# SJTU-ViSYS/Ground-Fusion

Measured on AMD Instinct MI355X. Metric: sliding-window solves/sec + tracked-features/sec, 640x480x10-frame window, higher is better.
Workload: dtype front end u8/s16 fixed point + f32; back end f64

## Files before the change

ground-fusion_amd/csrc/gf_ba.hip:

```cpp
#pragma clang fp contract(fast)
#include <hip/hip_runtime.h>
#include <algorithm>
#include <cmath>
#include <cstdio>
#include <cstdlib>
#include <cstring>
#include <atomic>
#include <memory>
#include <mutex>
#include <string>
#include <thread>
#include <vector>

#include "../../include/groundfusion_hip.h"
#include "gf_comm.hpp"
#include "gf_ba_kernels.hpp"
#include "gf_copy_list.hpp"
#include "gf_ba_marg.hpp"
#include "gf_ba_gnss.hpp"
#include "gf_hip_own.hpp"

using namespace gfb;

__global__ void ba_fill_plausible(void* p, size_t i0, size_t i1, int is_double, unsigned seed) {
// ... 658 lines not shown
}

int run_solve(gf_ba* h, int max_iters) {
    const Dims& d = h->d;
    const auto t_begin = std::chrono::steady_clock::now();
    if (int rc = launch_linearize(h, 0, 0, 0, false)) return rc;
    Win w = h->win();
    StepBufs sb = h->sbufs();
    const bool fuse_misc = h->fuse_misc && h->can_fuse_misc && d.GO == 0 && h->n_chain == 0;
    for (int it = 0; it <= max_iters; it++) {
        if (h->max_solver_time > 0.0 && it > 0 && it < max_iters) {
            HIPCHK(hipStreamSynchronize(h->stream));
            if (std::chrono::duration<double>(std::chrono::steady_clock::now() - t_begin).count() >= h->max_solver_time) it = max_iters;
        }
        poison_lds(h);
        const bool time_step = it == 1 && max_iters >= 1;
        if (time_step) HIPCHK(hipEventRecord(h->ev[6], h->stream));
        const int first = it == 0 ? 1 : 0, last = it == max_iters ? 1 : 0;
        const LaunchForm& ch = h->step_chain; const LaunchForm& de = h->step_dense;
        if (h->n_chain > 0) ch.fn<<<dim3(d.B), ch.threads, ch_lds_doubles(h->chain_nd) * sizeof(double), h->stream>>>(w, sb, first, max_iters, last);
        if (h->n_chain > 0 && h->n_dense == 0) { }
        else if (fuse_misc && it > 0 && h->step_waves != 4) ba_misc_step<<<dim3(d.B), 512, std::max(h->step_lds, h->mwin_lds), h->stream>>>(w, sb, max_iters, last);
        else de.fn<<<dim3(d.B), de.threads, de.lds, h->stream>>>(w, sb, first, max_iters, last);
        HIPCHK(hipGetLastError());
        if (time_step) { HIPCHK(hipEventRecord(h->ev[7], h->stream)); h->stats.step_launches++; h->stats.step_flops += h->step_flops; }
        if (it < max_iters) {
            const bool cost_only = h->cost_only && it == max_iters - 1 && it > 0 && d.GO == 0 && !h->split_jtj && !fuse_misc && !(h->max_solver_time > 0.0);
            if (int rc = launch_linearize(h, -1, -1, cost_only ? 3 : 1, it == 0, fuse_misc)) return rc;
            if (it == 0) { h->stats.jtj_launches++; h->stats.jtj_flops += h->mfma_per_lin * 2048; h->stats.jtj_alg_flops += h->jtj_alg_flops; }
        }
    }
    h->stats.solves += h->count;
    return GF_OK;
}

int run_marginalize(gf_ba* h, int mode) {
    const Dims& d = h->d;
    Win w = h->win();
    poison_lds(h);
    Win wm = w;
    wm.colf = h->mcolf[mode].d; wm.cole = h->mcole[mode].d; wm.order = h->morder[mode].d; wm.norder = h->mnorder[mode].d;
    if (mode == 0) { if (int rc = launch_visual(h, wm, true, -1, -2, 2)) return rc; }
    ba_linearize_misc_win<<<dim3(d.B), 64 * kMW, h->mwin_lds, h->stream>>>(wm, -1, -2, 2, mode == 0 ? 1 : 2);
    if (mode == 0 && d.GO) ba_linearize_gnss<<<dim3(d.B), 256, 0, h->stream>>>(wm, -1, -2, 2, 1);
    MargOut mo{h->outJ.d, h->outr.d};
    const double piv_eps = h->piv_eps;
    const int ls_rhs = h->ls_rhs;
    poison_lds(h);
    if (h->big_marg) ba_marg_finish<true><<<dim3(d.B), 512, 0, h->stream>>>(wm, h->sbufs(), reinterpret_cast<const MargInfo*>(h->minfo[mode].d), mo, mode == 0 ? 1 : 0, piv_eps, ls_rhs, 0);
    else ba_marg_finish<false><<<dim3(d.B), 512, h->marg_lds, h->stream>>>(wm, h->sbufs(), reinterpret_cast<const MargInfo*>(h->minfo[mode].d), mo, mode == 0 ? 1 : 0, piv_eps, ls_rhs, (int)(h->marg_lds / sizeof(double)));
    HIPCHK(hipGetLastError());
    return GF_OK;
}

}

extern "C" {

int gf_pose_subset_mask(int extrinsic_type) {
    switch (extrinsic_type) {
        case 0: return 0x00;
        case 2: return 0x07;
        case 3: return 0x04;
        case 4: return 0x3c;
        default: return 0x38;
    }
}

int gf_ba_create(const gf_ba_cfg* cfg, gf_ba** out) {
    if (!cfg || !out) return gf::set_err(GF_ERR_INVALID, "null argument");
    *out = nullptr;
    if (cfg->window_size < 2 || cfg->window_size > 30 || cfg->max_features < 1 || cfg->max_visual < 1 || cfg->batch < 1) return gf::set_err(GF_ERR_INVALID, "bad gf_ba_cfg");
    if (int rc = gf::require_device()) return rc;
    std::unique_ptr<gf_ba> h(new gf_ba());
    h->cfg = *cfg;
    Dims& d = h->d;
    d.B = cfg->batch; d.W = cfg->window_size; d.NP = d.W + 1; d.F = cfg->max_features; d.NV = cfg->max_visual;
    d.NVP = ((d.NV + d.NP * d.NP / 2 + 63) / 64) * 64;
    const bool gnss = cfg->max_gnss > 0;
    d.NG = gnss ? ((cfg->max_gnss + 63) & ~63) : 0; d.NGRP = gnss ? 4 * d.NP : 0;
    const int Rmax = 15 * d.NP + 17 + (gnss ? 5 * d.NP + 3 : 0);
    d.RP = (Rmax + 1 + 15) & ~15;  d.GO = gnss ? ((16 * d.NP + 20 + d.F + 3) & ~3) : 0; d.XS = gnss ? ((d.GO + 5 * d.NP + 4 + 3) & ~3) : ((16 * d.NP + 20 + d.F + 3) & ~3); d.NFB = 2 * d.NP + 7 + (gnss ? 5 * d.NP + 2 : 0); d.FP = (d.F + 3) & ~3; d.NPRI = d.RP; d.ECW = (6 * d.NP + 8 + 15) & ~15; d.NC = 6 * d.NP + 8; d.NVC = (d.NC * (d.NC + 1) / 2 + 3) & ~3;
    h->step_lds = (size_t)(Rmax + 1) * (Rmax + 2) / 2 * sizeof(double);
    h->big_step = h->step_lds + 27 * 1024 > 160 * 1024 || getenv("GF_BA_FORCE_GLOBAL") != nullptr;
    if (Rmax + 1 > 512) return gf::set_err(GF_ERR_INVALID, "window_size %d: reduced system (%d) exceeds 511 columns", d.W, Rmax);
    if (d.NV > 65535) return gf::set_err(GF_ERR_INVALID, "max_visual %d exceeds 65535", d.NV);
    if (misc_win_lds_doubles(d.W) * sizeof(double) > 160 * 1024)  return gf::set_err(GF_ERR_INVALID, "window_size %d: the IMU / wheel block rows exceed LDS (window_size <= 20 in this build)", d.W);
#define TRACED(x) do { g_alloc_what = #x; if (int rc_ = (x)) return rc_; } while (0)
    {
        int least = 0, greatest = 0;
        HIPCHK(hipDeviceGetStreamPriorityRange(&least, &greatest));
        const char* e = getenv("GF_BA_STREAM_PRIORITY");
        const int prio = (e && !strcmp(e, "default")) ? least + (greatest - least) / 2 : greatest;
        HIPCHK(hipStreamCreateWithPriority(&h->stream.s, hipStreamNonBlocking, prio));
    }
    for (auto& e : h->ev) HIPCHK(hipEventCreate(&e.e));
    HIPCHK(hipEventCreateWithFlags(&h->ev_gather.e, hipEventDisableTiming));
    HIPCHK(hipEventCreateWithFlags(&h->ev_gather_done.e, hipEventDisableTiming));
    const size_t B = d.B, VS = d.RP + d.FP;
    TRACED(h->xs0.alloc(B * d.XS, true)); TRACED(h->xs.alloc(2 * B * d.XS, true));
    TRACED(h->colf.alloc(B * d.NFB, true)); TRACED(h->cole.alloc(B * d.F, true)); TRACED(h->nvis.alloc(B, true)); TRACED(h->nimu.alloc(B, true)); TRACED(h->nwh.alloc(B, true)); TRACED(h->nfeat.alloc(B, true));
    TRACED(h->vis_idx.alloc(B * d.NV, true)); TRACED(h->vis_data.alloc(B * d.NV * 5, true)); TRACED(h->feat_obs.alloc(B * d.F * 6, true));
    TRACED(h->order.alloc(B * d.NVP, true)); TRACED(h->norder.alloc(B, true)); TRACED(h->feat_ptr.alloc(B * (d.F + 1), true)); TRACED(h->vis_pos.alloc(B * d.NV, true));
    TRACED(h->imu_i.alloc(B * d.W, true)); TRACED(h->imu_data.alloc(B * d.W * IMU_STRIDE2, true)); TRACED(h->wh_i.alloc(B * d.W, true)); TRACED(h->wh_data.alloc(B * d.W * WH_STRIDE, true));
    TRACED(h->pri_n.alloc(B, true)); TRACED(h->pri_nb.alloc(B, true)); TRACED(h->pri_bid.alloc(B * 64, true)); TRACED(h->pri_J.alloc(B * d.NPRI * d.NPRI, true));
    TRACED(h->pri_r.alloc(B * d.NPRI, true)); TRACED(h->pri_x0.alloc(B * d.NPRI * 2, true));
    HIPCHK(h->st.dev.alloc(B)); HIPCHK(h->st.pin.alloc(B)); h->st.view();
    HIPCHK(h->st0.dev.alloc(B)); HIPCHK(h->st0.pin.alloc(B)); h->st0.view();
    h->upload_kernel = !(getenv("GF_BA_UPLOAD") && !strcmp(getenv("GF_BA_UPLOAD"), "copies"));
    TRACED(h->imu_sqrt.alloc(B * d.W * 225, false)); TRACED(h->wh_sqrt.alloc(B * d.W * 36, false)); TRACED(h->pri_A.alloc(B * d.NPRI * d.NPRI, false)); TRACED(h->pri_b.alloc(B * d.NPRI, false));
    TRACED(h->pri_c.alloc(B, false)); TRACED(h->H.alloc(2 * B * d.RP * d.RP, true)); TRACED(h->g.alloc(2 * B * d.RP, true)); TRACED(h->Vc.alloc(2 * B * d.NVC, true)); TRACED(h->wpar.alloc(B * WPAR, true));
    TRACED(h->cost.alloc(6 * B, true)); TRACED(h->efac.alloc(B * d.NV * EF, false));
    HIPCHK(hipMemsetAsync(h->cost.d, 0, 6 * B * sizeof(double), h->stream));
    TRACED(h->scale.alloc(B * VS, false)); TRACED(h->diag.alloc(B * VS, false)); TRACED(h->grad.alloc(B * VS, false)); TRACED(h->gn.alloc(B * VS, false)); TRACED(h->step.alloc(B * VS, false));
    TRACED(h->u.alloc(B * VS, false)); TRACED(h->Et.alloc(2 * B * d.FP * d.ECW, true)); TRACED(h->Es.alloc(B * d.FP * d.ECW, false)); TRACED(h->ete.alloc(2 * B * d.FP, true)); TRACED(h->etb.alloc(2 * B * d.FP, true));
    TRACED(h->rhs.alloc(B * d.RP, false)); TRACED(h->yv.alloc(B * VS, false));
    if (gnss) { TRACED(h->ngnss.alloc(B, true)); TRACED(h->gn_idx.alloc(B * d.NG * 4, true)); TRACED(h->gn_data.alloc(B * d.NG * GN_STRIDE, true)); TRACED(h->gn_misc.alloc(B * (GN_MISC + d.NP), true)); TRACED(h->gn_gptr.alloc(B * (d.NGRP + 2), true)); TRACED(h->gn_gitem.alloc(B * d.NG, true)); TRACED(h->gn_rows.alloc(B * d.NG * GN_ROW, false)); }
    for (int m = 0; m < 2; m++) { TRACED(h->mcolf[m].alloc(B * d.NFB, true)); TRACED(h->mcole[m].alloc(B * d.F, true)); TRACED(h->morder[m].alloc(B * d.NVP, true)); TRACED(h->mnorder[m].alloc(B, true)); TRACED(h->minfo[m].alloc(B * 4, true)); }
    TRACED(h->minfo_stage.alloc(B * 4, true));
    TRACED(h->vpair.alloc(B * (size_t)(d.NP * (d.NP - 1) / 2) * VPG, false));
    TRACED(h->outJ.alloc(B * (size_t)d.NPRI * d.NPRI, true)); TRACED(h->outr.alloc(B * d.NPRI, true)); TRACED(h->stamps.alloc(128, true));
    const int nkeep = 6 * d.W + 9 + 17 + (gnss ? 9 : 0);
    h->big_marg = nkeep > 92 || getenv("GF_BA_FORCE_GLOBAL") != nullptr;
    h->meta.assign(d.B, gf_ba::SlotMeta{}); h->outJ_n.assign(d.B, 0); h->imu_dev.assign(d.B, 0); h->imu_rows.assign(d.B, 0);
    TRACED(h->imu_patch.alloc(B * d.W * IMU_STRIDE2, true)); TRACED(h->imu_pinfo.alloc(B * (d.W + 2), true));
    for (int mode = 0; mode < 2; mode++) h->keep_ids[mode].assign(d.B, {});
    h->marg_ncap = h->big_marg ? std::min(d.NPRI, nkeep + 16) : 92;
    h->marg_lds = h->big_marg ? 0 : (size_t)2 * h->marg_ncap * h->marg_ncap * sizeof(double);
    if (h->big_step) { h->sg_stride = (h->step_lds / sizeof(double) + 15) & ~(size_t)15; TRACED(h->Sg.alloc(B * h->sg_stride, false)); }
    if (h->big_marg) { h->mg_stride = (size_t)2 * h->marg_ncap * h->marg_ncap + 1024; TRACED(h->Mg.alloc(B * h->mg_stride, false)); }
    if (getenv("GF_BA_SPLIT_JTJ") && atoi(getenv("GF_BA_SPLIT_JTJ"))) if (int rc = gf_ba_set_split_jtj(h.get(), 1)) return rc;
    h->step_waves = (getenv("GF_BA_STEP_WAVES") && atoi(getenv("GF_BA_STEP_WAVES")) == 4) ? 4 : 8;
    h->chain_mode = getenv("GF_BA_CHAIN") && atoi(getenv("GF_BA_CHAIN")) != 0 && !h->big_step && !gnss;
    h->cost_only = !(getenv("GF_BA_COST_ONLY") && atoi(getenv("GF_BA_COST_ONLY")) == 0);
    h->piv_eps = getenv("GF_MARG_PIVOT_EPS") ? atof(getenv("GF_MARG_PIVOT_EPS")) : 3e-8;
    h->ls_rhs = getenv("GF_MARG_LS_RHS") ? atoi(getenv("GF_MARG_LS_RHS")) : 1;
    const int nd_max = Rmax - 9 * d.NP;
    if (h->chain_mode && ch_lds_doubles(nd_max) * sizeof(double) + 20 * 1024 > 160 * 1024) h->chain_mode = false;
    if (int rc = choose_launch_forms(h.get(), nd_max)) return rc;
    if (h->chain_mode) { h->yg_stride = ch_y_stride(nd_max); TRACED(h->Yg.alloc(B * d.NP * h->yg_stride, false)); }
    h->fuse_misc = getenv("GF_BA_FUSE_MISC") != nullptr;
    if (!h->vis_fixed.lds || !h->vis_free.lds) { h->vtile_stride = (vwin_slot_doubles(d.NP, true) + 3) & ~(size_t)3; TRACED(h->vtile.alloc(B * h->vtile_stride, false)); }
    h->mwin_lds = misc_win_lds_doubles(d.W) * sizeof(double);
    HIPCHK(hipFuncSetAttribute(reinterpret_cast<const void*>(ba_linearize_misc_win), hipFuncAttributeMaxDynamicSharedMemorySize, (int)h->mwin_lds));
    h->can_fuse_misc = !h->big_step && std::max(h->step_lds, h->mwin_lds) + 27 * 1024 <= 160 * 1024;
    if (h->can_fuse_misc) HIPCHK(hipFuncSetAttribute(reinterpret_cast<const void*>(ba_misc_step), hipFuncAttributeMaxDynamicSharedMemorySize, (int)std::max(h->step_lds, h->mwin_lds)));
    if (!h->big_marg) HIPCHK(hipFuncSetAttribute(reinterpret_cast<const void*>(ba_marg_finish<false>), hipFuncAttributeMaxDynamicSharedMemorySize, (int)h->marg_lds));
    HIPCHK(hipStreamSynchronize(h->stream));
#undef TRACED
    *out = h.release();
    return GF_OK;
}

int gf_ba_destroy(gf_ba* h) { delete h; return GF_OK; }

int gf_ba_upload(gf_ba* h, const gf_ba_window* windows, int count) {
    if (!h || !windows) return gf::set_err(GF_ERR_INVALID, "null argument");
    if (int rc = gf_ba_wait(h)) return rc;
    std::fill(h->outJ_n.begin(), h->outJ_n.end(), 0);
    if (int rc = pack_windows(h, windows, count)) return rc;
    h->resident.assign(count, nullptr);
    for (int b = 0; b < count; b++) h->resident[b] = windows + b;
    HIPCHK(hipEventRecord(h->ev[0], h->stream));
    if (int rc = upload(h)) return rc;
    HIPCHK(hipEventRecord(h->ev[1], h->stream));
    HIPCHK(hipStreamSynchronize(h->stream));
    float ms = 0; HIPCHK(hipEventElapsedTime(&ms, h->ev[0], h->ev[1])); h->stats.ms_upload += ms;
    return GF_OK;
}

int gf_ba_solve_resident_async(gf_ba* h, int max_iters, int marginalize_mode, int reset) {
    if (!h || h->count < 1) return gf::set_err(GF_ERR_INVALID, "no resident windows");
    if (h->pending) return gf::set_err(GF_ERR_INVALID, "a solve is already in flight: call gf_ba_wait first");
    if (max_iters < 0 || max_iters > 64) return gf::set_err(GF_ERR_INVALID, "max_iters out of range");
    if (marginalize_mode > 1) return gf::set_err(GF_ERR_INVALID, "marginalize_mode must be -1, 0 or 1");
    if (reset) { if (int rc = reset_state(h)) return rc; }
    HIPCHK(hipEventRecord(h->ev[0], h->stream));
    if (int rc = run_solve(h, max_iters)) return rc;
    HIPCHK(hipEventRecord(h->ev[1], h->stream));
    if (marginalize_mode >= 0) { if (int rc = run_marginalize(h, marginalize_mode)) return rc; h->last_marg_mode = marginalize_mode; }
    HIPCHK(hipEventRecord(h->ev[4], h->stream));
    h->pending = true; h->pending_iters = max_iters;
    return GF_OK;
}

int gf_ba_wait(gf_ba* h) {
    if (!h) return gf::set_err(GF_ERR_INVALID, "null handle");
    if (!h->pending) return GF_OK;
    HIPCHK(hipStreamSynchronize(h->stream));
    h->pending = false;
    float ms = 0;
    HIPCHK(hipEventElapsedTime(&ms, h->ev[0], h->ev[1])); h->stats.ms_solve += ms;
    HIPCHK(hipEventElapsedTime(&ms, h->ev[1], h->ev[4])); h->stats.ms_marginalize += ms;
    if (h->pending_iters > 0) { HIPCHK(hipEventElapsedTime(&ms, h->ev[2], h->ev[3])); h->stats.ms_jtj += ms; }
    if (h->pending_iters > 0 && h->split_timed) { HIPCHK(hipEventElapsedTime(&ms, h->ev_split[0], h->ev_split[1])); h->stats.ms_jtj_contract += ms; h->stats.jtj_contract_launches++; h->split_timed = false; }
    if (h->pending_iters > 0) { HIPCHK(hipEventElapsedTime(&ms, h->ev[6], h->ev[7])); h->stats.ms_step += ms; }
    return GF_OK;
}

int gf_ba_solve_resident(gf_ba* h, int max_iters, int marginalize_mode, int reset) {
    if (int rc = gf_ba_solve_resident_async(h, max_iters, marginalize_mode, reset)) return rc;
    return gf_ba_wait(h);
}


static int unpack_prior(gf_ba* h, int b, int mode, const double* x, gf_ba_prior& p) {
    const Dims& d = h->d;
    const int* inf = h->minfo[mode].h + (size_t)b * 4;
    p.valid = inf[3]; p.m = inf[0] + inf[1]; p.n = 0; p.nblocks = 0;
    if (!inf[3]) return GF_OK;
    const int n = inf[2];
    const std::vector<int>& keep = h->keep_ids[mode][b];
    if (n > p.cap_n || (int)keep.size() > p.cap_blocks) return gf::set_err(GF_ERR_CAPACITY, "prior capacity too small (n=%d, blocks=%zu)", n, keep.size());
    p.n = n; p.nblocks = (int)keep.size();
    if (p.J) memcpy(p.J, h->outJ.h + (size_t)b * d.NPRI * d.NPRI, (size_t)n * n * sizeof(double));
    memcpy(p.r, h->outr.h + (size_t)b * d.NPRI, (size_t)n * sizeof(double));
    int xo = 0;
    for (size_t q = 0; q < keep.size(); q++) {
        const int id = keep[q], kind = id / 4096, i = id % 4096;
        int nid = id;
        if (kind == GF_POSE || kind == GF_SPEEDBIAS || kind == GF_RCV_DDT) nid = mode == 0 ? kind * 4096 + i - 1 : (i == d.W ? kind * 4096 + d.W - 1 : id);
        else if (kind == GF_RCV_DT) nid = mode == 0 ? id - 4 : (i / 4 == d.W ? id - 4 : id);
        p.block_id[q] = nid;
        const int off = state_off_of(id, d);
        for (int k = 0; k < gsize_kind(kind); k++) p.x0[xo++] = x[off + k];
    }
    return GF_OK;
}
// ... 220 lines not shown
```

ground-fusion_amd/csrc/gf_ba_kernels.hpp:

```cpp
#pragma once
#include <type_traits>
#include <hip/hip_runtime.h>
#include <stdint.h>
#include "gf_dmath.hpp"

namespace gfb {
using namespace gfd;

typedef double d4 __attribute__((ext_vector_type(4)));

struct Dims {
    int B, W, NP, F, NV, NVP, RP, XS, NFB, FP, NPRI, ECW, GO, NG, NC, NVC, NGRP;
};
__host__ __device__ inline int off_pose(int i) { return 16 * i; }
__host__ __device__ inline int off_sb(int i) { return 16 * i + 7; }
__host__ __device__ inline int off_ex(int NP) { return 16 * NP; }
__host__ __device__ inline int off_exw(int NP) { return 16 * NP + 7; }
__host__ __device__ inline int off_ix(int NP) { return 16 * NP + 14; }
__host__ __device__ inline int off_td(int NP) { return 16 * NP + 17; }
__host__ __device__ inline int off_tdw(int NP) { return 16 * NP + 18; }
__host__ __device__ inline int off_feat(int NP) { return 16 * NP + 20; }
__host__ __device__ inline int fb_pose(int i) { return 2 * i; }
__host__ __device__ inline int fb_sb(int i) { return 2 * i + 1; }
__host__ __device__ inline int fb_ex(int NP) { return 2 * NP; }
// ... 1279 lines not shown
        a[J] = l;
        asm("" : "+v"(r));
        if (r == J) rd_own = rs;
        const double nlw = (r > J) ? -(l * rs) : 0.0;
        if (J > 0) Chol16W<J, 0>::fence(t);
        Chol16W<J, 0>::run(t, nlw);
        if (J < N - 1) {
            double nl = -l;
            dpp_fence(nl);
            Chol16A<J, J + 1, N>::run(a, nl, l);
        }
        Chol16Step<J + 1, N>::run(a, t, r, rd_own, good);
    }
};
template <int N> struct Chol16Step<N, N> { static __device__ __forceinline__ void run(double (&)[16], double (&)[4], int&, double&, bool&) {} };
template <class SPtr>
__device__ __forceinline__ bool wave_chol16_fused(SPtr S, int j0, int nb, double* s_inv, int lane) {
    int r = lane & 15;
    const int g = lane >> 4;
    double a[16], t[4];
    {
        const int base = pk(j0 + min(r, nb - 1), j0);
#pragma unroll
        for (int c = 0; c < 16; c++) a[c] = S[base + c];
        if (nb < 16) {
#pragma unroll
            for (int c = 0; c < 16; c++) a[c] = (r < nb && c < nb) ? a[c] : (r == c ? 1.0 : 0.0);
        }
    }
#pragma unroll
    for (int m = 0; m < 4; m++) t[m] = (4 * m + g == r) ? 1.0 : 0.0;
    double rd_own = 0.0;
    bool good = true;
    Chol16Step<0>::run(a, t, r, rd_own, good);
#pragma unroll
    for (int m = 0; m < 4; m++) {
        const int c = 4 * m + g;
        const double w = t[m] * rd_own;
        s_inv[r * 17 + c] = w;
        if (c <= r && r < nb) S[pk(j0 + r, j0 + c)] = w;
    }
    __builtin_amdgcn_fence(__ATOMIC_RELEASE, "wavefront"); __builtin_amdgcn_wave_barrier();
    return good;
}

__device__ __forceinline__ int ch_dm(int c, int NP) { return c < 15 * NP ? 6 * (c / 15) + (c % 15) : c - 9 * NP; }
__device__ __forceinline__ int ch_d2c(int dj, int NP) { return dj < 6 * NP ? 15 * (dj / 6) + dj % 6 : dj + 9 * NP; }
__device__ __forceinline__ bool ch_isv(int c, int NP) { return c < 15 * NP && (c % 15) >= 6; }
constexpr int kChPS = 13;
constexpr int kChYS = 9;
__host__ __device__ inline int ch_panel_rows(int ND) { return (ND + 1 + 15) & ~15; }
__host__ __device__ inline size_t ch_lds_doubles(int ND) { return (((size_t)(ND + 1) * (ND + 2) / 2 + 1) & ~(size_t)1) + 2 * (size_t)ch_panel_rows(ND) * kChPS + 3 * 272; }
__host__ __device__ inline size_t ch_y_stride(int ND) { return (size_t)ch_panel_rows(ND) * kChYS + 2 * 81; }
template <int NB, int LD>
__device__ __forceinline__ bool wave_chol_tile(const double* sA, double* s_inv, int lane) {
    int r = lane & 15;
    const int g = lane >> 4;
    double a[16], t[4];
    {
        const double* src = sA + min(r, NB - 1) * LD;
#pragma unroll
        for (int c = 0; c < 16; c++) a[c] = c < NB ? src[c] : 0.0;
#pragma unroll
        for (int c = 0; c < 16; c++) a[c] = (r < NB && c < NB) ? a[c] : (r == c ? 1.0 : 0.0);
    }
#pragma unroll
    for (int m = 0; m < 4; m++) t[m] = (4 * m + g == r) ? 1.0 : 0.0;
    double rd_own = 1.0;
    bool good = true;
    Chol16Step<0, NB>::run(a, t, r, rd_own, good);
#pragma unroll
    for (int m = 0; m < 4; m++) s_inv[r * 17 + 4 * m + g] = t[m] * rd_own;
    __builtin_amdgcn_fence(__ATOMIC_RELEASE, "wavefront"); __builtin_amdgcn_wave_barrier();
    return good;
}

template <bool GS, int NW = 8, bool CH = false>
__device__ __forceinline__ void ba_step_body(Win w, StepBufs sb, int first, int max_iters, int finalize_only) {
    static_assert(!(CH && GS), "the chain form keeps its dense part in LDS");
    extern __shared__ __attribute__((aligned(16))) double smem[];
    constexpr int NRC = CH ? 256 : 512;
    constexpr int NCC = CH ? 96 : 256;
    __shared__ double sred[512];
    __shared__ double s_inv[16 * 17];
    __shared__ double s_y[32];
    __shared__ int s_flag[4];
    __shared__ int s_cmap[NCC];
    __shared__ double s_uc[NCC];
    __shared__ double s_ucc[NCC];
    __shared__ double s_rd[NRC];
    __shared__ int s_rc[NRC];
    __shared__ double s_hd[NRC];
    __shared__ double s_gt[NRC];
    __shared__ double s_yd[CH ? 96 : 1];
    constexpr int NT = 64 * NW;
    const Dims d = w.d;
    const int b = blockIdx.x, tid = threadIdx.x, wave = tid >> 6, lane = tid & 63;
    SolverState& st = w.st[b];
    if (uni(st.done)) return;
    if ((uni(st.chain) != 0) != CH) return;
    const int R = uni(st.R), NE = uni(st.NE), RP = d.RP, VS = sb.VS, ECW = d.ECW;
    double* S = GS ? sb.Sg + (size_t)blockIdx.x * sb.SgStride : smem;
    const int CNP = d.NP, ND = CH ? R - 9 * CNP : R, RC = CH ? ND : R;
#define DMAP(c) (CH ? ch_dm((c), CNP) : (c))
    const int* colf = w.colf + (size_t)b * d.NFB;
    const int* cole = w.cole + (size_t)b * d.F;
    double* scale = sb.scale + (size_t)b * VS; double* diag = sb.diag + (size_t)b * VS; double* grad = sb.grad + (size_t)b * VS;
    double* gn = sb.gn + (size_t)b * VS; double* stepv = sb.step + (size_t)b * VS; double* u = sb.u + (size_t)b * VS; double* yv = sb.yv + (size_t)b * VS;
    double* Es = sb.Es + (size_t)b * d.FP * ECW;
    if (tid < ECW) s_cmap[tid] = compact_to_col(tid, colf, d.NP, R);
    for (int q = tid; q < NRC; q += NT) s_rc[q] = -1;
    __syncthreads();
    if (tid < 6 * d.NP + 7) { const int c = s_cmap[tid]; if (c >= 0 && c < R) s_rc[c] = tid; }
    GF_STAMP(0);
    if (tid == 0) {
        s_flag[0] = 0;
        if (first) {
            st.x_cost = cost_total(w, st.cur, b);
            st.initial_cost = st.x_cost;
            st.last_successful = 1;
        } else if (st.cand_valid) {
            const double cand_cost = cost_total(w, 1 - st.cur, b);
            st.cand_cost = cand_cost;
            if (st.step_norm <= 1e-8 * (st.x_norm + 1e-8)) { st.done = 1; st.termination = 2; }
            else if (fabs(st.x_cost - cand_cost) <= 1e-6 * st.x_cost) { st.done = 1; st.termination = 1; }
            else {
                const double rel = (st.x_cost - cand_cost) / st.model_cost_change;
                if (rel > 1e-3) {
                    st.cur = 1 - st.cur; st.x_cost = cand_cost; st.successful++; st.last_successful = 1; s_flag[0] = 1;
                    if (rel < 0.25) st.radius *= 0.5;
                    if (rel > 0.75) st.radius = fmax(st.radius, 3.0 * st.dogleg_step_norm);
                    st.mu = fmax(1e-8, 2.0 * st.mu / 10.0);
                    st.reuse = 0;
                } else { st.radius *= 0.5; st.reuse = 1; st.last_successful = 0; }
            }
        }
    }
    __syncthreads();
    if (uni(st.done)) return;
    const int cur = uni(st.cur);
    double* H = w.H + ((size_t)cur * d.B + b) * RP * RP;
    double* g = w.g + ((size_t)cur * d.B + b) * RP;
    const double* xs = w.xs + ((size_t)cur * d.B + b) * d.XS;
    const double* Et = sb.Et + ((size_t)cur * d.B + b) * d.FP * ECW;
    const double* ete = sb.ete + ((size_t)cur * d.B + b) * d.FP;
    const double* etb = sb.etb + ((size_t)cur * d.B + b) * d.FP;
    const double* Vc = w.Vc + ((size_t)cur * d.B + b) * d.NVC;
    const int RHSK = 6 * d.NP + 7;
    for (int c = tid; c < R; c += NT) {
        const int k = s_rc[c];
        s_hd[c] = H[(size_t)c * RP + c] + (k >= 0 ? Vc[pk(k, k)] : 0.0);
        s_gt[c] = g[c] + (k >= 0 ? Vc[pk(RHSK, k)] : 0.0);
    }
    __syncthreads();
    GF_STAMP(1);
    if (!uni(st.reuse)) {
        if (!st.have_scale) {
            for (int c = tid; c < R; c += NT) scale[c] = 1.0 / (1.0 + sqrt(s_hd[c]));
            for (int e = tid; e < NE; e += NT) scale[RP + e] = 1.0 / (1.0 + sqrt(ete[e]));
            __syncthreads();
            if (tid == 0) st.have_scale = 1;
        }
        double gm = 0;
        for (int c = tid; c < R; c += NT) gm = fmax(gm, fabs(s_gt[c]));
        for (int e = tid; e < NE; e += NT) gm = fmax(gm, fabs(etb[e]));
        gm = block_max<NW>(gm, sred, tid, NT);
        if (tid == 0) st.gmax = gm;
// ... 284 lines not shown
                for (int k = CNP - 1; k >= 0; k--) {
                    const int par = (CNP - 1 - k) & 1;
                    double* Pc = Pb0 + (size_t)par * PR * kChPS;
                    double* Pp = Pb0 + (size_t)(par ^ 1) * PR * kChPS;
                    double* sA = sA0 + 136 * par; double* sC = sC0 + 136 * par;
                    if (k < CNP - 1) {
                        const int ft = ftile(k + 1);
                        for (int t = ft + uw; t <= NTD; t += NW) {
                            d4 acc = {0, 0, 0, 0};
                            const double* pa = t < NTD ? Pp + (size_t)(16 * t + ti_) * kChPS + kq_ : sE + ti_ * 17 + kq_;
                            const double* pb = sE + ti_ * 17 + kq_;
                            const double a0 = pa[0], a1 = pa[4], a2 = pa[8], b0 = pb[0], b1 = pb[4], b2 = pb[8];
                            double c0[4];
                            if (ti_ < 9) {
#pragma unroll
                                for (int r = 0; r < 4; r++) { const int row = kq_ + 4 * r; c0[r] = t < NTD ? Pc[(size_t)(16 * t + row) * kChPS + ti_] : (row < 9 ? sA[row * 15 + ti_] : 0.0); }
                            }
                            acc = __builtin_amdgcn_mfma_f64_16x16x4f64(a0, b0, acc, 0, 0, 0);
                            acc = __builtin_amdgcn_mfma_f64_16x16x4f64(a1, b1, acc, 0, 0, 0);
                            acc = __builtin_amdgcn_mfma_f64_16x16x4f64(a2, b2, acc, 0, 0, 0);
                            if (ti_ < 9) {
#pragma unroll
                                for (int r = 0; r < 4; r++) {
                                    const int row = kq_ + 4 * r;
                                    if (t < NTD) Pc[(size_t)(16 * t + row) * kChPS + ti_] = c0[r] - acc[r];
                                    else if (row < 9) sA[row * 15 + ti_] = c0[r] - acc[r];
                                }
                            }
                        }
                        dense_update(Pp, ft);
                    }
                    __syncthreads();
                    GF_CQ(0);
                    if (uw == 0) {
                        __builtin_amdgcn_s_setprio(3);
                        const bool good = wave_chol_tile<9, 15>(sA, s_inv, lane);
                        if (!good && lane == 0) s_flag[1] = 0;
                        __builtin_amdgcn_s_setprio(0);
                    } else if (k >= 1) {
                        for (int q = t3; q < PR * 9; q += NTF) { const int rr = q / 9; Pp[(size_t)rr * kChPS + q - 9 * rr] = 0.0; }
                    }
                    __syncthreads();
                    GF_CQ(1);
                    if (!uni(s_flag[1])) break;
                    double* Yk = Yg + (size_t)k * sb.YgStride;
                    for (int t = ftile(k) + uw; t <= NTD; t += NW) {
                        d4 acc = {0, 0, 0, 0};
                        double a0, a1, a2;
                        if (t < NTD) { const double* pa = Pc + (size_t)(16 * t + ti_) * kChPS + kq_; a0 = pa[0]; a1 = pa[4]; a2 = pa[8]; }
                        else { const int i9 = min(ti_, 8); a0 = sC[kq_ * 15 + i9]; a1 = sC[(kq_ + 4) * 15 + i9]; a2 = kq_ == 0 ? sC[8 * 15 + i9] : 0.0; if (ti_ >= 9) { a0 = 0.0; a1 = 0.0; a2 = 0.0; } }
                        const double* pb = s_inv + ti_ * 17 + kq_;
                        const double b0 = pb[0], b1 = pb[4], b2 = pb[8];
                        acc = __builtin_amdgcn_mfma_f64_16x16x4f64(a0, b0, acc, 0, 0, 0);
                        acc = __builtin_amdgcn_mfma_f64_16x16x4f64(a1, b1, acc, 0, 0, 0);
                        acc = __builtin_amdgcn_mfma_f64_16x16x4f64(a2, b2, acc, 0, 0, 0);
                        if (ti_ < 9) {
#pragma unroll
                            for (int r = 0; r < 4; r++) {
                                const int row = kq_ + 4 * r;
                                if (t < NTD) { Pc[(size_t)(16 * t + row) * kChPS + ti_] = acc[r]; Yk[(size_t)(16 * t + row) * kChYS + ti_] = acc[r]; }
                                else if (row < 9) { sE[row * 17 + ti_] = acc[r]; Yk[(size_t)PR * kChYS + 81 + row * 9 + ti_] = acc[r]; }
                            }
                        }
                    }
                    if (tid < 81) Yk[(size_t)PR * kChYS + tid] = s_inv[(tid / 9) * 17 + tid % 9];
                    if (k >= 2) { if (t3 >= 0) { front_store(k - 1, Pp, sA0 + 136 * (par ^ 1), sC0 + 136 * (par ^ 1)); if (k >= 3) front_load(k - 2); } }
                    else if (k == 1) front0_gather(Pp, sA0 + 136 * (par ^ 1));
                    __syncthreads();
                    GF_CQ(2);
                }
#ifdef GF_PROFILE_STEP
                if (blockIdx.x == 0 && tid == 0 && sb.stamps) { sb.stamps[87] = cq[0]; sb.stamps[88] = cq[1]; sb.stamps[89] = cq[2]; sb.stamps[90] = clock64(); }
#endif
                if (uni(s_flag[1])) dense_update(Pb0 + (size_t)((CNP - 1) & 1) * PR * kChPS, 0);
                __syncthreads();
            }
#ifdef GF_PROFILE_STEP
            long long tA = 0, tB = 0, tC = 0, t0c = clock64();
            if (blockIdx.x == 0 && tid == 0 && sb.stamps) { sb.stamps[24] = sb.stamps[25] = sb.stamps[26] = sb.stamps[27] = sb.stamps[28] = sb.stamps[29] = sb.stamps[30] = sb.stamps[31] = 0; }
#define GF_SUB(acc) do { const long long n_ = clock64(); acc += n_ - t0c; t0c = n_; } while (0)
#else
#define GF_SUB(acc) do { } while (0)
#endif
            auto diag_block = [&](int j0) {
                const int nb = min(16, RC - j0);
#ifdef GF_PROFILE_STEP
                long long d0 = clock64();
#define GF_DSUB(i) do { const long long n_ = clock64(); if (blockIdx.x == 0 && tid == 0 && sb.stamps) sb.stamps[i] += n_ - d0; d0 = n_; } while (0)
#else
#define GF_DSUB(i) do { } while (0)
#endif
                GF_DSUB(24);
                const bool good = wave_chol16_fused(S, j0, nb, s_inv, lane);
                GF_DSUB(25);
                GF_DSUB(26);
                if (!good && lane == 0) s_flag[1] = 0;
                GF_DSUB(27);
            };
            const int NTR = (RC + 16) / 16;
            auto upd_tile = [&](int ti, int tj, int k0, int k1) {
                const int ra = 16 * ti + (lane & 15), rb = 16 * tj + (lane & 15), kq = lane >> 4;
                const bool va = ra <= RC, vb = rb < RC;
                const int base_a = pk(min(ra, RC), 0) + kq, base_b = pk(min(rb, RC - 1), 0) + kq;
                d4 acc0 = {0, 0, 0, 0}, acc1 = {0, 0, 0, 0};
                if (k0 >= k1) return;
#pragma unroll 2
                for (int k = k0; k < k1; k++) {
                    double av[4], bv2[4];
#pragma unroll
                    for (int q = 0; q < 4; q++) { av[q] = S[base_a + 16 * k + 4 * q]; bv2[q] = S[base_b + 16 * k + 4 * q]; }
#pragma unroll
                    for (int q = 0; q < 4; q++) { av[q] = va ? av[q] : 0.0; bv2[q] = vb ? bv2[q] : 0.0; }
                    acc0 = __builtin_amdgcn_mfma_f64_16x16x4f64(av[0], bv2[0], acc0, 0, 0, 0);
                    acc1 = __builtin_amdgcn_mfma_f64_16x16x4f64(av[1], bv2[1], acc1, 0, 0, 0);
                    acc0 = __builtin_amdgcn_mfma_f64_16x16x4f64(av[2], bv2[2], acc0, 0, 0, 0);
                    acc1 = __builtin_amdgcn_mfma_f64_16x16x4f64(av[3], bv2[3], acc1, 0, 0, 0);
                }
#pragma unroll
                for (int r = 0; r < 4; r++) {
                    const int row = 16 * ti + (lane >> 4) + 4 * r, col = 16 * tj + (lane & 15);
                    if (row <= RC && col <= row && col < RC) S[pk(row, col)] -= acc0[r] + acc1[r];
                }
            };
            const bool chain_ok = !CH || uni(s_flag[1]) != 0;
            for (int j0 = 0; j0 < RC && chain_ok; j0 += 16) {
                const int nb = min(16, RC - j0), jb = j0 >> 4;
#ifdef GF_PROFILE_STEP
                const long long w0c = clock64();
#endif
                if (wave == 0) {
                    __builtin_amdgcn_s_setprio(3);
                    if (jb > 0) { upd_tile(jb, jb, jb - 1, jb); __builtin_amdgcn_fence(__ATOMIC_RELEASE, "wavefront"); __builtin_amdgcn_wave_barrier(); }
                    diag_block(j0);
                    __builtin_amdgcn_s_setprio(0);
                } else {
                    if (jb > 0) for (int t = wave; t < NTR - jb; t += NW - 1) upd_tile(jb + t, jb, 0, jb);
                    if (wave == NW - 1 && jb + 1 < NTR && 16 * (jb + 1) < RC) upd_tile(jb + 1, jb + 1, 0, jb);
                }
#ifdef GF_PROFILE_STEP
                if (blockIdx.x == 0 && sb.stamps && (tid == 0 || tid == 64 || tid == 256) && jb < 12) sb.stamps[(tid == 0 ? 40 : tid == 64 ? 56 : 72) + jb] = clock64() - w0c;
#endif
                __syncthreads();
                GF_SUB(tC);
                if (!uni(s_flag[1])) break;
                const int r0 = j0 + nb;
                auto panel = [&](auto full) {
                    constexpr bool FULL = decltype(full)::value;
                    const int nrows = RC + 1 - r0, nt = (nrows + 15) / 16;
                    for (int t = wave; t < nt; t += NW) {
                        const int ra = r0 + 16 * t + (lane & 15);
                        const int rb_ = pk(min(ra, RC), j0);
                        d4 acc = {0, 0, 0, 0};
#pragma unroll
                        for (int k = 0; k < 4; k++) {
                            const int kc = 4 * k + (lane >> 4);
                            const double av = (ra <= RC && (FULL || kc < nb)) ? S[rb_ + kc] : 0.0;
                            const double bv2 = s_inv[(lane & 15) * 17 + kc];
                            acc = __builtin_amdgcn_mfma_f64_16x16x4f64(av, bv2, acc, 0, 0, 0);
                        }
                        __builtin_amdgcn_wave_barrier();
#pragma unroll
                        for (int r = 0; r < 4; r++) {
                            const int row = r0 + 16 * t + (lane >> 4) + 4 * r, c = lane & 15;
                            if (row <= RC && (FULL || c < nb)) S[pk(row, j0 + c)] = acc[r];
                        }
                    }
                };
                if (nb == 16) panel(std::true_type{}); else panel(std::false_type{});
                __syncthreads();
                GF_SUB(tB);
            }
#ifdef GF_PROFILE_STEP
            if (blockIdx.x == 0 && tid == 0 && sb.stamps) { sb.stamps[20] = tA; sb.stamps[21] = tB; sb.stamps[22] = tC; }
#endif
            ok = uni(s_flag[1]) != 0;
            if (ok) {
                GF_STAMP(9);
                for (int r = tid; r < RC; r += NT) s_rd[r] = 0.0;
                __syncthreads();
                for (int j0 = ((RC - 1) / 16) * 16, par = 0; j0 >= 0; j0 -= 16, par ^= 1) {
                    const int nb = min(16, RC - j0);
#ifdef GF_PROFILE_STEP
                    const long long bq0 = clock64();
#endif
                    if (wave == 0) {
                        __builtin_amdgcn_s_setprio(3);
                        const int cc = lane & 15, lz = min(lane, nb - 1);
                        double z = S[pk(RC, j0 + lz)] + s_rd[j0 + lz];
                        z = lane < nb ? z : 0.0;
                        double wc[16];
                        double lnext[16];
                        const int rn = max(j0 - 16, 0) + cc;
                        if (nb == 16) {
#pragma unroll
                            for (int rr = 0; rr < 16; rr++) { const double v = S[pk(j0 + rr, j0) + min(cc, rr)]; wc[rr] = cc <= rr ? v : 0.0; }
#pragma unroll
                            for (int c = 0; c < 16; c++) lnext[c] = S[pk(j0 + c, 0) + rn];
                        } else {
#pragma unroll
                            for (int rr = 0; rr < 16; rr++) {
                                const int rl = min(rr, nb - 1);
                                const double v = S[pk(j0 + rl, j0 + min(cc, rl))];
                                wc[rr] = (rr < nb && cc <= rr) ? v : 0.0;
                            }
#pragma unroll
                            for (int c = 0; c < 16; c++) lnext[c] = S[pk(j0 + min(c, nb - 1), rn)];
                        }
                        const double zn = S[pk(RC, rn)];
                        double y0 = 0.0, y1 = 0.0;
#pragma unroll
                        for (int rr = 0; rr < 16; rr += 2) { y0 += wc[rr] * row_bcast(z, rr); y1 += wc[rr + 1] * row_bcast(z, rr + 1); }
                        z = y0 + y1;
                        if (lane < nb) { s_y[16 * par + lane] = z; if (CH) s_yd[j0 + lane] = z; else yv[j0 + lane] = z; }
                        if (lane >= nb && lane < 16) s_y[16 * par + lane] = 0.0;
                        if (j0 > 0) {
                            double sv = zn;
#pragma unroll
                            for (int c = 0; c < 16; c++) sv -= lnext[c] * row_bcast(z, c);
                            if (lane < 16) S[pk(RC, rn)] = sv;
                        }
                        __builtin_amdgcn_s_setprio(0);
                    }
#ifdef GF_PROFILE_STEP
                    const long long bq1 = clock64();
#endif
                    __syncthreads();
#ifdef GF_PROFILE_STEP
                    const long long bq2 = clock64();
                    if (blockIdx.x == 0 && tid == 0 && sb.stamps) { sb.stamps[29] += bq1 - bq0; sb.stamps[30] += bq2 - bq1; }
                    if (blockIdx.x == 0 && tid == 64 && sb.stamps) { sb.stamps[31] += bq2 - bq1; }
#endif
                    if (wave > 0) {
                        const double* yb = s_y + 16 * par;
                        for (int r = tid - 64; r < j0 - 16; r += NT - 64) {
                            double lv[16];
#pragma unroll
                            for (int c = 0; c < 16; c++) lv[c] = c < nb ? S[pk(j0 + c, r)] : 0.0;
                            double acc = 0.0;
#pragma unroll
                            for (int c = 0; c < 16; c++) acc += lv[c] * yb[c];
                            s_rd[r] -= acc;
                        }
                    }
                }
                __syncthreads();
#ifdef GF_PROFILE_STEP
                if (CH && blockIdx.x == 0 && tid == 0 && sb.stamps) sb.stamps[91] = clock64();
#endif
                if (CH) {
                    const int PR = ch_panel_rows(ND);
                    double* sWE = smem + ((((size_t)(ND + 1) * (ND + 2) / 2) + 1) & ~(size_t)1);
// ... 207 lines not shown
```

Measured before the change: 97480.

## Pipeline blocked Cholesky with look-ahead diagonal factor and register-fused panel updates

Restructures the in-LDS blocked Cholesky of the reduced system into a look-ahead schedule. Wave 0 computes the next column's panel tile, updates it and factors the next diagonal block into a double-buffered inverse. The other waves keep their panel results in registers and apply the rank-16 trailing update straight from them, so each column needs one barrier instead of two and fewer LDS round trips. The price is an extra 16x17 inverse buffer in shared memory (the LDS budget thresholds rise from 27 to 28 KiB), a fixed row-to-wave ownership that may balance work less evenly, and more intricate synchronisation through sred.

```diff
diff --git a/ground-fusion_amd/csrc/gf_ba.hip b/ground-fusion_amd/csrc/gf_ba.hip
--- a/ground-fusion_amd/csrc/gf_ba.hip
+++ b/ground-fusion_amd/csrc/gf_ba.hip
@@ -764,7 +764,7 @@
     const int Rmax = 15 * d.NP + 17 + (gnss ? 5 * d.NP + 3 : 0);
     d.RP = (Rmax + 1 + 15) & ~15;  d.GO = gnss ? ((16 * d.NP + 20 + d.F + 3) & ~3) : 0; d.XS = gnss ? ((d.GO + 5 * d.NP + 4 + 3) & ~3) : ((16 * d.NP + 20 + d.F + 3) & ~3); d.NFB = 2 * d.NP + 7 + (gnss ? 5 * d.NP + 2 : 0); d.FP = (d.F + 3) & ~3; d.NPRI = d.RP; d.ECW = (6 * d.NP + 8 + 15) & ~15; d.NC = 6 * d.NP + 8; d.NVC = (d.NC * (d.NC + 1) / 2 + 3) & ~3;
     h->step_lds = (size_t)(Rmax + 1) * (Rmax + 2) / 2 * sizeof(double);
-    h->big_step = h->step_lds + 27 * 1024 > 160 * 1024 || getenv("GF_BA_FORCE_GLOBAL") != nullptr;
+    h->big_step = h->step_lds + 28 * 1024 > 160 * 1024 || getenv("GF_BA_FORCE_GLOBAL") != nullptr;
     if (Rmax + 1 > 512) return gf::set_err(GF_ERR_INVALID, "window_size %d: reduced system (%d) exceeds 511 columns", d.W, Rmax);
     if (d.NV > 65535) return gf::set_err(GF_ERR_INVALID, "max_visual %d exceeds 65535", d.NV);
     if (misc_win_lds_doubles(d.W) * sizeof(double) > 160 * 1024)  return gf::set_err(GF_ERR_INVALID, "window_size %d: the IMU / wheel block rows exceed LDS (window_size <= 20 in this build)", d.W);
@@ -825,7 +825,7 @@
     if (!h->vis_fixed.lds || !h->vis_free.lds) { h->vtile_stride = (vwin_slot_doubles(d.NP, true) + 3) & ~(size_t)3; TRACED(h->vtile.alloc(B * h->vtile_stride, false)); }
     h->mwin_lds = misc_win_lds_doubles(d.W) * sizeof(double);
     HIPCHK(hipFuncSetAttribute(reinterpret_cast<const void*>(ba_linearize_misc_win), hipFuncAttributeMaxDynamicSharedMemorySize, (int)h->mwin_lds));
-    h->can_fuse_misc = !h->big_step && std::max(h->step_lds, h->mwin_lds) + 27 * 1024 <= 160 * 1024;
+    h->can_fuse_misc = !h->big_step && std::max(h->step_lds, h->mwin_lds) + 28 * 1024 <= 160 * 1024;
     if (h->can_fuse_misc) HIPCHK(hipFuncSetAttribute(reinterpret_cast<const void*>(ba_misc_step), hipFuncAttributeMaxDynamicSharedMemorySize, (int)std::max(h->step_lds, h->mwin_lds)));
     if (!h->big_marg) HIPCHK(hipFuncSetAttribute(reinterpret_cast<const void*>(ba_marg_finish<false>), hipFuncAttributeMaxDynamicSharedMemorySize, (int)h->marg_lds));
     HIPCHK(hipStreamSynchronize(h->stream));
diff --git a/ground-fusion_amd/csrc/gf_ba_kernels.hpp b/ground-fusion_amd/csrc/gf_ba_kernels.hpp
--- a/ground-fusion_amd/csrc/gf_ba_kernels.hpp
+++ b/ground-fusion_amd/csrc/gf_ba_kernels.hpp
@@ -1385,7 +1385,7 @@
     constexpr int NRC = CH ? 256 : 512;
     constexpr int NCC = CH ? 96 : 256;
     __shared__ double sred[512];
-    __shared__ double s_inv[16 * 17];
+    __shared__ double s_inv[2 * 16 * 17];
     __shared__ double s_y[32];
     __shared__ int s_flag[4];
     __shared__ int s_cmap[NCC];
@@ -1836,7 +1836,7 @@
 #else
 #define GF_SUB(acc) do { } while (0)
 #endif
-            auto diag_block = [&](int j0) {
+            auto diag_block = [&](int j0, double* inv_out) {
                 const int nb = min(16, RC - j0);
 #ifdef GF_PROFILE_STEP
                 long long d0 = clock64();
@@ -1845,19 +1845,20 @@
 #define GF_DSUB(i) do { } while (0)
 #endif
                 GF_DSUB(24);
-                const bool good = wave_chol16_fused(S, j0, nb, s_inv, lane);
+                const bool good = wave_chol16_fused(S, j0, nb, inv_out, lane);
                 GF_DSUB(25);
                 GF_DSUB(26);
                 if (!good && lane == 0) s_flag[1] = 0;
                 GF_DSUB(27);
             };
             const int NTR = (RC + 16) / 16;
-            auto upd_tile = [&](int ti, int tj, int k0, int k1) {
-                const int ra = 16 * ti + (lane & 15), rb = 16 * tj + (lane & 15), kq = lane >> 4;
+            const int li = lane & 15, kq = lane >> 4;
+            auto upd_tile = [&](int ti, int tj, int k0, int k1, const double* xa = nullptr, const double* xb = nullptr) {
+                const int ra = 16 * ti + li, rb = 16 * tj + li;
                 const bool va = ra <= RC, vb = rb < RC;
                 const int base_a = pk(min(ra, RC), 0) + kq, base_b = pk(min(rb, RC - 1), 0) + kq;
                 d4 acc0 = {0, 0, 0, 0}, acc1 = {0, 0, 0, 0};
-                if (k0 >= k1) return;
+                if (k0 >= k1 && !xa) return;
 #pragma unroll 2
                 for (int k = k0; k < k1; k++) {
                     double av[4], bv2[4];
@@ -1870,57 +1871,100 @@
                     acc0 = __builtin_amdgcn_mfma_f64_16x16x4f64(av[2], bv2[2], acc0, 0, 0, 0);
                     acc1 = __builtin_amdgcn_mfma_f64_16x16x4f64(av[3], bv2[3], acc1, 0, 0, 0);
                 }
+                if (xa) {
+                    double av[4], bv2[4];
+#pragma unroll
+                    for (int q = 0; q < 4; q++) { av[q] = va ? xa[q] : 0.0; bv2[q] = vb ? xb[q] : 0.0; }
+                    acc0 = __builtin_amdgcn_mfma_f64_16x16x4f64(av[0], bv2[0], acc0, 0, 0, 0);
+                    acc1 = __builtin_amdgcn_mfma_f64_16x16x4f64(av[1], bv2[1], acc1, 0, 0, 0);
+                    acc0 = __builtin_amdgcn_mfma_f64_16x16x4f64(av[2], bv2[2], acc0, 0, 0, 0);
+                    acc1 = __builtin_amdgcn_mfma_f64_16x16x4f64(av[3], bv2[3], acc1, 0, 0, 0);
+                }
 #pragma unroll
                 for (int r = 0; r < 4; r++) {
-                    const int row = 16 * ti + (lane >> 4) + 4 * r, col = 16 * tj + (lane & 15);
+                    const int row = 16 * ti + kq + 4 * r, col = 16 * tj + li;
                     if (row <= RC && col <= row && col < RC) S[pk(row, col)] -= acc0[r] + acc1[r];
                 }
             };
+            auto panel_op = [&](auto full, int rbase, int j0, int nb, const double* inv, double (&x)[4]) {
+                constexpr bool FULL = decltype(full)::value;
+                const int ra = rbase + li, rb_ = pk(min(ra, RC), j0);
+                d4 acc = {0, 0, 0, 0};
+#pragma unroll
+                for (int k = 0; k < 4; k++) {
+                    const int kc = 4 * k + kq;
+                    const double av = (ra <= RC && (FULL || kc < nb)) ? S[rb_ + kc] : 0.0;
+                    const double bv2 = inv[li * 17 + kc];
+                    acc = __builtin_amdgcn_mfma_f64_16x16x4f64(bv2, av, acc, 0, 0, 0);
+                }
+#pragma unroll
+                for (int q = 0; q < 4; q++) x[q] = acc[q];
+            };
+            auto panel_store = [&](auto full, int rbase, int j0, int nb, const double (&x)[4]) {
+                constexpr bool FULL = decltype(full)::value;
+                const int ra = rbase + li, rb_ = pk(min(ra, RC), j0);
+#pragma unroll
+                for (int q = 0; q < 4; q++) if (ra <= RC && (FULL || 4 * q + kq < nb)) S[rb_ + 4 * q + kq] = x[q];
+            };
             const bool chain_ok = !CH || uni(s_flag[1]) != 0;
+            auto owner = [&](int i) -> int { return 1 + (i - 1) % (NW - 1); };
+            if (chain_ok) {
+                if (wave == 0) { __builtin_amdgcn_s_setprio(3); diag_block(0, s_inv); __builtin_amdgcn_s_setprio(0); }
+                __syncthreads();
+                GF_SUB(tC);
+            }
             for (int j0 = 0; j0 < RC && chain_ok; j0 += 16) {
+                if (!uni(s_flag[1])) break;
                 const int nb = min(16, RC - j0), jb = j0 >> 4;
 #ifdef GF_PROFILE_STEP
                 const long long w0c = clock64();
 #endif
+                const int r0 = j0 + nb;
+                const double* inv = s_inv + 272 * (jb & 1);
+                const bool next_col = nb == 16 && r0 < RC;
                 if (wave == 0) {
-                    __builtin_amdgcn_s_setprio(3);
-                    if (jb > 0) { upd_tile(jb, jb, jb - 1, jb); __builtin_amdgcn_fence(__ATOMIC_RELEASE, "wavefront"); __builtin_amdgcn_wave_barrier(); }
-                    diag_block(j0);
-                    __builtin_amdgcn_s_setprio(0);
+                    if (next_col) {
+                        __builtin_amdgcn_s_setprio(3);
+                        double x[4];
+                        panel_op(std::true_type{}, r0, j0, 16, inv, x);
+                        upd_tile(jb + 1, jb + 1, 0, 0, x, x);
+                        __builtin_amdgcn_fence(__ATOMIC_RELEASE, "wavefront"); __builtin_amdgcn_wave_barrier();
+                        diag_block(r0, s_inv + 272 * ((jb + 1) & 1));
+                        __builtin_amdgcn_s_setprio(0);
+                    }
                 } else {
-                    if (jb > 0) for (int t = wave; t < NTR - jb; t += NW - 1) upd_tile(jb + t, jb, 0, jb);
-                    if (wave == NW - 1 && jb + 1 < NTR && 16 * (jb + 1) < RC) upd_tile(jb + 1, jb + 1, 0, jb);
+                    if (jb > 0 && owner(jb) == wave) {
+                        double xh[4];
+#pragma unroll
+                        for (int q = 0; q < 4; q++) xh[q] = sred[256 * ((jb - 1) & 1) + 64 * q + lane];
+                        panel_store(std::true_type{}, j0, j0 - 16, 16, xh);
+                    }
+                    double xb[4] = {0, 0, 0, 0};
+                    if (next_col) panel_op(std::true_type{}, r0, j0, 16, inv, xb);
+                    const int nt = (RC + 1 - r0 + 15) / 16;
+                    auto rows = [&](auto full) {
+                        for (int t = 0; t < nt; t++) {
+                            const int i = jb + 1 + t;
+                            if (owner(i) != wave) continue;
+                            double xa[4];
+                            if (t == 0 && next_col) {
+#pragma unroll
+                                for (int q = 0; q < 4; q++) sred[256 * (jb & 1) + 64 * q + lane] = xb[q];
+                                continue;
+                            }
+                            panel_op(full, r0 + 16 * t, j0, nb, inv, xa);
+                            panel_store(full, r0 + 16 * t, j0, nb, xa);
+                            if (next_col) {
+                                upd_tile(i, jb + 1, 0, jb, xa, xb);
+                                if (t == 1 && 16 * (jb + 2) < RC) upd_tile(i, i, 0, jb, xa, xa);
+                            }
+                        }
+                    };
+                    if (nb == 16) rows(std::true_type{}); else rows(std::false_type{});
                 }
 #ifdef GF_PROFILE_STEP
                 if (blockIdx.x == 0 && sb.stamps && (tid == 0 || tid == 64 || tid == 256) && jb < 12) sb.stamps[(tid == 0 ? 40 : tid == 64 ? 56 : 72) + jb] = clock64() - w0c;
 #endif
-                __syncthreads();
-                GF_SUB(tC);
-                if (!uni(s_flag[1])) break;
-                const int r0 = j0 + nb;
-                auto panel = [&](auto full) {
-                    constexpr bool FULL = decltype(full)::value;
-                    const int nrows = RC + 1 - r0, nt = (nrows + 15) / 16;
-                    for (int t = wave; t < nt; t += NW) {
-                        const int ra = r0 + 16 * t + (lane & 15);
-                        const int rb_ = pk(min(ra, RC), j0);
-                        d4 acc = {0, 0, 0, 0};
-#pragma unroll
-                        for (int k = 0; k < 4; k++) {
-                            const int kc = 4 * k + (lane >> 4);
-                            const double av = (ra <= RC && (FULL || kc < nb)) ? S[rb_ + kc] : 0.0;
-                            const double bv2 = s_inv[(lane & 15) * 17 + kc];
-                            acc = __builtin_amdgcn_mfma_f64_16x16x4f64(av, bv2, acc, 0, 0, 0);
-                        }
-                        __builtin_amdgcn_wave_barrier();
-#pragma unroll
-                        for (int r = 0; r < 4; r++) {
-                            const int row = r0 + 16 * t + (lane >> 4) + 4 * r, c = lane & 15;
-                            if (row <= RC && (FULL || c < nb)) S[pk(row, j0 + c)] = acc[r];
-                        }
-                    }
-                };
-                if (nb == 16) panel(std::true_type{}); else panel(std::false_type{});
                 __syncthreads();
                 GF_SUB(tB);
             }
```

New measurement: 95320. 0.978x the previous value.
